# boromir674/relation-autoencoder

Measured on NVIDIA B200. Metric: AC-model train examples/sec, higher is better.
Workload: dtype f32

## Files before the change

### relation_autoencoder_b200/csrc/rae_decoder_tc.cu

```cuda
#include <cuda_fp16.h>
#include <stdlib.h>

#include <algorithm>
#include <vector>

#include "rae_common.cuh"
#include "rae_internal.h"

namespace rae {

namespace {

#ifdef RAE_TRACE
__device__ unsigned long long* g_tc_trace = nullptr;
__device__ int g_tc_knock = 0;
#define TC_KNOCK(bit) ((g_tc_knock & (bit)) != 0)
#define TC_TRACE_INIT() unsigned long long* const tc_trace_ptr_ = g_tc_trace
#define TC_TRACE_INIT_IF(cond) unsigned long long* const tc_trace_ptr_ = (cond) ? g_tc_trace : nullptr
#define TC_TRACE(slot)                                                                                         \
    do {                                                                                                       \
        if (tc_trace_ptr_ != nullptr && (slot) < 64) tc_trace_ptr_[(size_t)blockIdx.x * 64 + (slot)] = clock64(); \
    } while (0)
#define TC_TRACE_NS(slot)                                                                                      \
    do {                                                                                                       \
// ... 168 lines not shown
    asm volatile("tcgen05.st.sync.aligned.32x32b.x4.b32 [%0], {%1, %2, %3, %4};" ::"r"(taddr), "r"(v[0]), "r"(v[1]), "r"(v[2]), "r"(v[3])
                 : "memory");
}
__host__ __device__ __forceinline__ float pow2_scale(uint32_t amax_bits) {
    const int e = (int)((amax_bits >> 23) & 255u) - 127;
    if (((amax_bits >> 23) & 255u) == 0u) return 1.f;
    int se = 11 - e;
    se = se < -100 ? -100 : (se > 100 ? 100 : se);
    union { uint32_t u; float f; } cv;
    cv.u = (uint32_t)(se + 127) << 23;
    return cv.f;
}
constexpr float TC_QSCALE = 4096.f;
enum TcScal { TS_AMAX_C = 0, TS_AMAX_L = 1, TS_AMAX_R = 2, TS_AMAX_A = 3, TS_AMAX_CV = 4, TS_AMAX_Y2 = 5, TS_N = 8 };

__device__ __forceinline__ float ldg_stream(const float* p) {
    float v;
    asm volatile("ld.global.nc.f32 %0, [%1];" : "=f"(v) : "l"(p));
    return v;
}

__device__ __forceinline__ float ldg_ordered(const float* p) {
    float v;
    asm volatile("ld.global.f32 %0, [%1];" : "=f"(v) : "l"(p) : "memory");
    return v;
}

struct TcSeg { int tile, u0, u1, slot; };
struct TcSegIter {
    TcSched s; long long cur, end; int x;
    __device__ __forceinline__ TcSegIter(TcSched s_, int x_) : s(s_), cur(tcs_start(s_, x_)), end(tcs_start(s_, x_ + 1)), x(x_) {}
    __device__ __forceinline__ bool next(TcSeg& g) {
        if (cur >= end) return false;
        g.tile = (int)(cur / s.upt);
        g.u0 = (int)(cur - (long long)g.tile * s.upt);
        const long long len = min((long long)(s.upt - g.u0), end - cur);
        g.u1 = g.u0 + (int)len;
        g.slot = x - tcs_first(s, g.tile);
        cur += len;
        return true;
    }
};

__device__ __forceinline__ const float* cf_row(const float* C, const float* C1, const float* C2, int d, int K, int DP,
                                               int n_bil_rows, int n) {
    if (n < n_bil_rows) {
        const int i = n / DP, j = n - i * DP;
        return (i < d && j < d && C != nullptr) ? C + ((size_t)i * d + j) * K : nullptr;
    }
    const int m = n - n_bil_rows;
    const int which = m / DP, j = m - which * DP;
    if (j >= d || which > 1) return nullptr;
    const float* src = which == 0 ? C1 : C2;
    return src != nullptr ? src + (size_t)j * K : nullptr;
}

__global__ void __launch_bounds__(256) k_tc_absmax(const float* __restrict__ C, size_t nC, const float* __restrict__ C1, size_t n1,
                                                   const float* __restrict__ C2, size_t n2, uint32_t* __restrict__ out) {
    pdl_enter();
    __shared__ uint32_t red[8];
    uint32_t m = 0;
    const size_t stride = (size_t)gridDim.x * blockDim.x, t0 = (size_t)blockIdx.x * blockDim.x + threadIdx.x;
    auto scan = [&](const float* p, size_t n) {
        if (p == nullptr || n == 0) return;
        if ((n & 3) == 0 && (reinterpret_cast<uintptr_t>(p) & 15) == 0) {
            const float4* p4 = reinterpret_cast<const float4*>(p);
// ... 377 lines not shown
                        for (int x = 0; x < 32; ++x)
                            if (jb + x < p.d) o[(size_t)(jb + x) * p.B] = inv * t[x];
                    }
                }
                if (DP >= 64 && bil && ok && i0 < p.d) p.vT[((size_t)g * p.dp + i0) * p.B + b] = inv * vsum;
                if (etr) TC_TRACE(56);
            }
            if (ok) {
                float* wo = p.wT + ((size_t)sg.slot * 2 + g) * p.dp * p.B + b;
#pragma unroll
                for (int c = 0; c < RW; ++c) {
                    const int j = jbase + c;
                    if (j < p.dp) wo[(size_t)j * p.B] = inv * Wr[c];
                }
            }
            if (ew == 0 && lane == 0 && it <= (sg.u1 - sg.u0)) TC_TRACE(9);
        }
        if (ew == 0 && lane == 0) TC_TRACE(4);
    }
    tc_fence_before();
    __syncthreads();
    if (threadIdx.x == 0) { TC_TRACE(5); TC_TRACE_NS(15); }
    if (warp == TC_FWD_WORKERS + 2) {
        tc_fence_after();
        asm volatile("tcgen05.dealloc.cta_group::1.sync.aligned.b32 %0, %1;" ::"r"(tmem_base), "r"(512u) : "memory");
    }
}

constexpr uint32_t TC_BWD_ACOL = 128;
constexpr int TC_DQ_ASTAGES = 3;
constexpr int TC_DC_ASTAGES = 2;
constexpr uint32_t TC_BWD_ACC2 = 384;
constexpr int TC_DC_MAX_STAGES = 16;
constexpr int TC_DQ_MAX_STAGES = 64;

constexpr int TC_IMG_LD = 68;
struct TrJob { const float* src; size_t stride; int cols, cols_out; float* dst; uint32_t* amax; int img; };
struct TrJobs { TrJob j[4]; int B; };
__global__ void __launch_bounds__(256) k_tc_transpose(TrJobs jobs) {
    pdl_enter();
    __shared__ float tile[32][33];
    __shared__ uint32_t red[8];
    const TrJob jb = jobs.j[blockIdx.z];
    const int b0 = blockIdx.x * 32, c0 = blockIdx.y * 32;
    if (c0 >= jb.cols_out) return;
    const int tx = threadIdx.x & 31, ty = threadIdx.x >> 5;
    uint32_t m = 0;
    for (int r = ty; r < 32; r += 8) {
        const int b = b0 + r, c = c0 + tx;
        const float v = (b < jobs.B && c < jb.cols) ? jb.src[(size_t)b * jb.stride + c] : 0.f;
        tile[r][tx] = v;
        m = max(m, __float_as_uint(fabsf(v)));
    }
    if (jb.amax != nullptr) {
#pragma unroll
        for (int o = 16; o > 0; o >>= 1) m = max(m, __shfl_xor_sync(kFull, m, o));
        if (tx == 0) red[ty] = m;
    }
    __syncthreads();
    for (int r = ty; r < 32; r += 8) {
        const int c = c0 + r, b = b0 + tx;
        if (c < jb.cols_out && b < jobs.B) {
            if (jb.img) jb.dst[((size_t)(b >> 6) * jb.cols_out + c) * TC_IMG_LD + (b & 63)] = tile[tx][r];
            else jb.dst[(size_t)c * jobs.B + b] = tile[tx][r];
        }
    }
    if (jb.amax != nullptr && threadIdx.x == 0) {
// ... 127 lines not shown
            tc_commit(&br.b_empty[s]);
            if (lt == nst - 1) tc_commit(br.acc_full);
        }
        __syncwarp();
        if ((threadIdx.x & 31) == 0 && git == 8) TC_TRACE(trace_base + 7);
        if ((threadIdx.x & 31) == 0 && git == 24) TC_TRACE(trace_base + 12);
    }
}

__device__ __forceinline__ void bwd_store8(uint32_t lane_base, int as, int col8, const float (&g)[8]) {
    float hi[8], lo[8];
    split8(g, hi, lo);
    const uint32_t col = lane_base + TC_BWD_ACOL + 128u * as + (uint32_t)col8;
    tc_st8(col, hi);
    tc_st8(col + 64u, lo);
}
__device__ __forceinline__ void bwd_publish(const BwdBars& br, int as, int lane) {
    tc_wait_st();
    tc_fence_before();
    __syncwarp();
    if (lane == 0) mbar_arrive(&br.a_full[as]);
}

struct TcDqArgs {
    const uint4* bop2;
    const float* sc;
    const float* aT; const float* LT; const float* RT; const float* cT; const float* Y2T;
    float* dqT;
    const uint32_t* scal;
    float g_bound;
    int B, d, dp, K, NK;
    int n_bil_rows;
    TcSched sch;
};

__device__ __forceinline__ void dq_mma_segment(const BwdBars& br, uint8_t* smB, uint32_t ST_BYTES, int NK, uint32_t tmem_base, int nst,
                                               int it0) {
    TC_TRACE_INIT();
    constexpr int NAS = TC_DQ_ASTAGES;
    const uint32_t idesc = make_idesc_f16(TC_M, NK);
    bool ready = false;
    for (int lt = 0; lt < nst; ++lt) {
        const int git = it0 + lt, s = git % TC_BSTAGES, as = git % NAS;
        if (!ready) {
            mbar_wait(&br.a_full[as], (git / NAS) & 1);
            mbar_wait(&br.b_full[s], (git / TC_BSTAGES) & 1);
            tc_fence_after();
        }
        ready = false;
        if (git == 8) TC_TRACE(22);
        if (git == 24) TC_TRACE(27);
        const uint32_t a_hi = tmem_base + TC_BWD_ACOL + 128u * as, a_lo = a_hi + 64u;
        const uint32_t b_base = smem_u32(smB + (size_t)s * ST_BYTES);
        uint64_t dbh = make_desc(b_base, (uint32_t)NK * 16u, 128u);
        uint64_t dbl = make_desc(b_base + 16u * (uint32_t)NK * 16u, (uint32_t)NK * 16u, 128u);
#pragma unroll
        for (int ks = 0; ks < 8; ++ks) {
            if (TC_KNOCK(2)) continue;
            if (ks == 4 && lt + 1 < nst) {
                const int g1 = git + 1;
                mbar_wait(&br.a_full[g1 % NAS], (g1 / NAS) & 1);
                mbar_wait(&br.b_full[g1 % TC_BSTAGES], (g1 / TC_BSTAGES) & 1);
                tc_fence_after();
                ready = true;
            }
            tc_mma_f16_ts(tmem_base, a_hi + 8u * ks, dbh, idesc, (lt > 0 || ks > 0) ? 1u : 0u);
// ... 9 lines not shown
        if (git == 24) TC_TRACE(28);
    }
}

__device__ __forceinline__ void dq_store16(uint32_t lane_base, int as, int col8, const float (&g)[16]) {
    uint32_t hi[8], lo[8];
#pragma unroll
    for (int u = 0; u < 8; ++u) split_h2(g[2 * u], g[2 * u + 1], hi[u], lo[u]);
    const uint32_t col = lane_base + TC_BWD_ACOL + 128u * as + (uint32_t)col8;
    tc_st8u(col, hi);
    tc_st8u(col + 64u, lo);
}

template <int DP>
__global__ void __launch_bounds__(TC_BWD_THREADS, 1) k_tc_dq(TcDqArgs p) {
    pdl_enter();
    extern __shared__ __align__(128) uint8_t smem_raw[];
    const int warp = threadIdx.x >> 5, lane = threadIdx.x & 31;
    TC_TRACE_INIT();
    constexpr int NAS = TC_DQ_ASTAGES;
    constexpr int RPS = 128 / DP;
    const uint32_t ST_BYTES = 2u * 16u * (uint32_t)p.NK * 16u;
    uint8_t* smB = smem_raw;
    uint32_t tmem_base;
    if (threadIdx.x == 0) { TC_TRACE(16); TC_TRACE_NS(30); }
    const BwdBars br = bwd_setup(smem_raw, ST_BYTES, warp, tmem_base);
    if (threadIdx.x == 0) TC_TRACE(17);

    if (warp >= TC_BWD_WORKERS) {
        asm volatile("setmaxnreg.dec.sync.aligned.u32 32;" ::: "memory");
    }
    if (warp == TC_BWD_WORKERS + 1) {
        if (lane == 0) {
            TcSegIter si(p.sch, blockIdx.x);
            TcSeg sg;
            int it = 0;
            while (si.next(sg)) {
                bwd_produce(br, smB, reinterpret_cast<const uint8_t*>(p.bop2), ST_BYTES, sg.u0, sg.u1 - sg.u0, it);
                it += sg.u1 - sg.u0;
            }
        }
    } else if (warp == TC_BWD_WORKERS) {
        if (elect_one()) {
            TcSegIter si(p.sch, blockIdx.x);
            TcSeg sg;
            int it = 0, seg = 0;
            while (si.next(sg)) {
                if (seg > 0) {
                    mbar_wait(br.acc_empty, (seg - 1) & 1);
                    tc_fence_after();
                }
                dq_mma_segment(br, smB, ST_BYTES, p.NK, tmem_base, sg.u1 - sg.u0, it);
                it += sg.u1 - sg.u0;
                ++seg;
            }
            TC_TRACE(19);
        }
        __syncwarp();
    } else if (warp < TC_BWD_WORKERS) {
        asm volatile("setmaxnreg.inc.sync.aligned.u32 112;" ::: "memory");
        const int gw = warp, q4 = gw & 3, cg = gw >> 2;
        const int row = q4 * 32 + lane;
        const uint32_t lane_base = tmem_base + ((uint32_t)(q4 * 32) << 16);
        const int rsel = (32 * cg) / DP, j0 = (32 * cg) % DP;
        const int n_bil_st = p.n_bil_rows / TC_M;
        float sG, inv;
        {
            const float aL = __uint_as_float(p.scal[TS_AMAX_L]), aR = __uint_as_float(p.scal[TS_AMAX_R]);
            const float aA = __uint_as_float(p.scal[TS_AMAX_A]), aC = __uint_as_float(p.scal[TS_AMAX_CV]);
            const float aY = __uint_as_float(p.scal[TS_AMAX_Y2]);
            const float bound = fmaxf(fmaf(aA, aR, aL * aY), fmaxf(fmaf(p.g_bound, aL, aA), fmaf(p.g_bound, aR, aC)));
            sG = pow2_scale(__float_as_uint(bound));
            inv = 1.f / (sG * pow2_scale(p.scal[TS_AMAX_C]));
        }
        TcSegIter si(p.sch, blockIdx.x);
        TcSeg sg;
        int it = 0, seg = 0;
        while (si.next(sg)) {
            const int b = sg.tile * TC_M + row;
            const bool ok = b < p.B;
            const float* scb = p.sc + (size_t)(ok ? b : 0) * SC_N;
            float X[32], Y[32];
            {
                const float* rp = p.RT + (ok ? b : 0);
                const float* yp = p.Y2T + (ok ? b : 0);
                const int jlast = p.dp - 1;
#pragma unroll
                for (int u = 0; u < 32; ++u) {
                    X[u] = ldg_stream(rp + (size_t)min(j0 + u, jlast) * p.B);
                    Y[u] = ldg_stream(yp + (size_t)min(j0 + u, jlast) * p.B);
                }
#pragma unroll
                for (int u = 0; u < 32; ++u)
                    if (!(ok && j0 + u < p.dp)) { X[u] = 0.f; Y[u] = 0.f; }
            }
            if (gw == 0 && lane == 0 && it == 0 && X[0] != -1.f) TC_TRACE(29);
            const int st0 = sg.u0, st1 = sg.u1, nst = st1 - st0;
            const int nbil = max(0, min(st1, n_bil_st) - st0);
            float ai_n = 0.f, li_n = 0.f;
            {
                const int i = RPS * st0 + rsel;
                if (nbil > 0 && ok && i < p.dp) {
                    ai_n = p.aT[(size_t)i * p.B + b];
                    li_n = p.LT[(size_t)i * p.B + b];
                }
            }
            int lt = 0;
            for (; lt < nbil; ++lt) {
// ... 686 lines not shown
    for (int j = lane; j < d; j += 32) {
        o[E_L * dp + j] = ld_nc(A + (size_t)r1 * d + j);
        o[E_R * dp + j] = ld_nc(A + (size_t)r2 * d + j);
    }
}
}

int tc_supported(const rae_engine* h) {
    if (!h->hasM) return 0;
    if (h->d <= 16 || h->d > 128) return 0;
    if (h->K > 104) return 0;
    return 1;
}

int tc_init(rae_engine* h) {
    const int DP = tc_dp(h->d);
    TcState& t = h->tc;
    t.DP = DP;
    t.KH = (h->K + 15) & ~15;
    const int rps = 128 / DP;
    const int di = (h->d + rps - 1) / rps * rps;
    t.n_bil_rows = di * DP;
    t.n_bil_half = t.n_bil_rows / TC_H;
    t.n_sp_half = h->hasSP ? (2 * DP) / TC_H : 0;
    t.n_rows_total = (t.n_bil_rows + (h->hasSP ? 2 * DP : 0) + TC_M - 1) / TC_M * TC_M;
    t.n_chunks_fwd = (t.n_bil_half + t.n_sp_half + 1) / 2;
    t.n_chunks_rec = t.n_bil_half / 2;
    t.ntile = (h->B + TC_M - 1) / TC_M;
    const size_t b_bytes = (size_t)2 * (t.KH / 8) * TC_N * 16;
    t.fwd_stages = (int)std::min<size_t>(4, ((size_t)h->max_smem_optin - 256) / b_bytes);
    if (t.fwd_stages < 2) return fail(h, RAE_EINVAL, "tensor path: K=%d needs %zu bytes per operand stage, two do not fit", h->K, b_bytes);
    t.smem = (size_t)t.fwd_stages * b_bytes + 256;
    t.sch_fwd = make_sched(t.ntile, t.n_chunks_fwd, h->num_sms, 0);
    t.sch_rec = make_sched(t.ntile, t.n_chunks_rec, h->num_sms, 0);
    t.slots_vw = std::max(sched_max_slots(t.sch_fwd), sched_max_slots(t.sch_rec));
    t.NK = (h->K + 15) & ~15;
    const int n_st = t.n_rows_total / TC_M;
    t.sch_dq = make_sched(t.ntile, n_st, h->num_sms, TC_DQ_MAX_STAGES);
    t.slots_dq = sched_max_slots(t.sch_dq);
    const size_t st_bytes = (size_t)2 * 2 * 8 * t.NK * 16;
    t.smem_dq = (size_t)TC_BSTAGES * st_bytes + 256;
    if (t.smem_dq > (size_t)h->max_smem_optin) return fail(h, RAE_EINVAL, "tensor path: backward operand stages do not fit in shared memory");
    t.n_ntiles = t.n_rows_total / TC_M;
    t.n_bst = (h->B + TC_SR - 1) / TC_SR;
    t.dc_nacc = 2;
    const size_t per_stage = (size_t)(TC_M / DP) * 2 * TC_SR * sizeof(float);
    const int cap = (int)(((size_t)h->max_smem_optin - t.smem_dq) / per_stage);
    if (cap < 1) return fail(h, RAE_EINVAL, "tensor path: no shared memory left for the dC staging area");
    const int n_bil_tiles = t.n_bil_rows / TC_M;
    t.dc2 = (h->B % 4 == 0) && n_bil_tiles > 0;
    t.smem_dc2 = (size_t)TC_DC2_BSTAGES * (2 * 8 * t.NK * 16) + (size_t)TC_DC2_XSTAGES * (2 * (size_t)DP * TC_IMG_LD * 4 + 2 * (TC_M / DP) * 2 * 256) + 256;
    if (t.smem_dc2 > (size_t)h->max_smem_optin) t.dc2 = false;
    t.dc_tile0 = t.dc2 ? n_bil_tiles : 0;
    t.slots_dc = 1;
    if (t.dc2) {
        t.sch_dc2 = make_sched((n_bil_tiles + 1) / 2, t.n_bst, h->num_sms, TC_DC2_MAX_STAGES);
        t.slots_dc = sched_max_slots(t.sch_dc2);
    }
    t.dc_tiles = t.n_ntiles - t.dc_tile0;
    if (t.dc_tiles > 0) {
        t.sch_dc = make_sched(t.dc_tiles, t.n_bst, h->num_sms, std::min(t.dc_nacc * TC_DC_MAX_STAGES, cap));
        t.dc_share = sched_max_share(t.sch_dc);
        t.slots_dc = std::max(t.slots_dc, sched_max_slots(t.sch_dc));
    }
    t.smem_dc = t.smem_dq + (size_t)t.dc_share * per_stage;
    cudaError_t e;
    const size_t vec = (size_t)h->dp * h->B * sizeof(float);
    if ((e = cudaMalloc((void**)&t.bop, (size_t)t.n_chunks_fwd * b_bytes)) != cudaSuccess ||
        (e = cudaMalloc((void**)&t.vT, 2 * vec)) != cudaSuccess ||
        (e = cudaMalloc((void**)&t.wT, 2 * t.slots_vw * vec)) != cudaSuccess ||
        (e = cudaMalloc((void**)&t.spT, 2 * vec)) != cudaSuccess ||
// ... 90 lines not shown
                                                              h->quirk ? 1 : 0, h->ev, t.scal, reinterpret_cast<uint4*>(t.pop4));
    h->launches++;
    RAE_CUDA(h, cudaGetLastError());
    const int slots[2] = {E_L, E_R};
    float* const dst[2] = {t.LT, t.RT};
    const int words[2] = {TS_AMAX_L, TS_AMAX_R};
    return tc_transpose_slots(h, 2, slots, dst, words, true, E_R, t.Rimg, st);
}

int tc_prepare_qt(rae_engine* h, cudaStream_t st) {
    TcState& t = h->tc;
    const int nbc = 2 * t.n_bst;
    const size_t total3 = (size_t)nbc * 8 * t.NK;
    const int blocks3 = (int)std::min<size_t>((total3 + 255) / 256, (size_t)h->num_sms * 8);
    launch_pdl(k_tc_prep_qt, dim3(blocks3, 1), dim3(256), 0, st, h->q, h->B, h->K, t.NK, nbc, t.pop3, h->P[RAE_P_A], nullptr, nullptr, h->d, h->dp,
                                                   h->quirk ? 1 : 0, h->ev, t.scal, nullptr);
    h->launches++;
    RAE_CUDA(h, cudaGetLastError());
    return RAE_OK;
}

int tc_contract(rae_engine* h, const float* LT_in, const float* RT_in, int slotV, int slotW, bool with_sp, cudaStream_t st) {
    TcState& t = h->tc;
    TcArgs p{};
    p.qT = t.qT; p.bop = t.bop; p.LT = LT_in; p.RT = RT_in; p.spT = t.spT; p.vT = t.vT; p.wT = t.wT; p.scal = t.scal;
    p.B = h->B; p.K = h->K; p.d = h->d; p.dp = h->dp; p.KH = t.KH;
    p.n_bil_half = t.n_bil_half; p.n_sp_half = with_sp ? t.n_sp_half : 0;
    p.nbs = t.fwd_stages;
    p.sch = with_sp ? t.sch_fwd : t.sch_rec;
    if (t.DP == 32) launch_pdl(k_tc_bilinear<32>, dim3(p.sch.G), dim3(TC_FWD_THREADS), t.smem, st, p);
    else if (t.DP == 64) launch_pdl(k_tc_bilinear<64>, dim3(p.sch.G), dim3(TC_FWD_THREADS), t.smem, st, p);
    else launch_pdl(k_tc_bilinear<128>, dim3(p.sch.G), dim3(TC_FWD_THREADS), t.smem, st, p);
    RAE_CUDA(h, cudaGetLastError());
    launch_pdl(k_tc_combine, dim3((h->B + 31) / 32, (h->d + 31) / 32), dim3(256), 0, st, t.vT, t.wT, (with_sp && h->hasSP) ? t.spT : nullptr, h->ev, h->B, h->d,
                                                                          h->dp, t.DP, p.sch, slotV, slotW, with_sp ? t.scal : nullptr);
    h->launches += 2;
    RAE_CUDA(h, cudaGetLastError());
    return RAE_OK;
}

int tc_forward(rae_engine* h, cudaStream_t st) { return tc_contract(h, h->tc.LT, h->tc.RT, E_V1, E_V2, true, st); }

int tc_backward_recompute(rae_engine* h, cudaStream_t st) {
    TcState& t = h->tc;
    const int slots[3] = {E_A, E_CV, E_Y2};
    float* const dst[3] = {t.aT, t.cT, t.Y2T};
    const int words[3] = {TS_AMAX_A, TS_AMAX_CV, TS_AMAX_Y2};
    int rc = tc_transpose_slots(h, 3, slots, dst, words, false, E_Y2, t.Yimg, st);
    if (rc) return rc;
    return tc_contract(h, t.aT, t.cT, E_GA1, E_GA2, false, st);
}

int tc_backward_dq(rae_engine* h, cudaStream_t st) {
    TcState& t = h->tc;
    TcDqArgs p{};
    p.bop2 = reinterpret_cast<const uint4*>(t.bop2); p.sc = h->sc; p.aT = t.aT; p.LT = t.LT; p.RT = t.RT; p.cT = t.cT; p.Y2T = t.Y2T;
    p.dqT = t.dqT; p.scal = t.scal; p.g_bound = (float)((double)h->S / h->Z);
    p.B = h->B; p.d = h->d; p.dp = h->dp; p.K = h->K; p.NK = t.NK;
    p.n_bil_rows = t.n_bil_rows;
    p.sch = t.sch_dq;
    if (t.DP == 32) launch_pdl(k_tc_dq<32>, dim3(p.sch.G), dim3(TC_BWD_THREADS), t.smem_dq, st, p);
    else if (t.DP == 64) launch_pdl(k_tc_dq<64>, dim3(p.sch.G), dim3(TC_BWD_THREADS), t.smem_dq, st, p);
    else launch_pdl(k_tc_dq<128>, dim3(p.sch.G), dim3(TC_BWD_THREADS), t.smem_dq, st, p);
    h->launches += 1;
    RAE_CUDA(h, cudaGetLastError());
    return RAE_OK;
}

int tc_backward_finish(rae_engine* h, cudaStream_t st) {
    TcState& t = h->tc;
    const int blocks = (h->B + 31) / 32;
    if (blocks > h->n_dz_part) return fail(h, RAE_EINVAL, "internal: dzsum_part too small");
    h->dz_part_used = blocks;
    const size_t smem = sizeof(float) * 32 * ((size_t)(h->K | 1) + h->K);
    launch_pdl(k_tc_bwd_finish, dim3(blocks), dim3(1024), smem, st, h->ev, h->sc, h->q, h->logq, t.dqT, h->dz, h->dzsum_part, h->B, h->K, t.NK, t.sch_dq,
                                               h->d, h->dp, h->hasSP ? 1 : 0, (float)(2.0 * h->cfg.alpha / h->Z));
    h->launches += 1;
    RAE_CUDA(h, cudaGetLastError());
    return RAE_OK;
}

int tc_grad_dense(rae_engine* h, cudaStream_t st) {
    TcState& t = h->tc;
    if (t.dc2) {
        TcDc2Args p{};
        p.pop4 = reinterpret_cast<const uint4*>(t.pop4); p.Rimg = t.Rimg; p.Yimg = t.Yimg; p.aT = t.aT; p.LT = t.LT; p.out = h->gC_part;
        p.scal = t.scal; p.g_bound = (float)((double)h->S / h->Z);
        p.B = h->B; p.d = h->d; p.dp = h->dp; p.K = h->K; p.NK = t.NK; p.DP = t.DP;
        p.n_bil_tiles = t.n_bil_rows / TC_M;
        p.split_stride = (size_t)h->off_gWb;
        p.sch = t.sch_dc2;
        launch_pdl(k_tc_dc2, dim3(p.sch.G), dim3(TC_BWD_THREADS), t.smem_dc2, st, p);
        h->launches++;
        RAE_CUDA(h, cudaGetLastError());
    }
    if (t.dc_tiles > 0) {
// ... 391 lines not shown
```

### relation_autoencoder_b200/csrc/rae_engine.cu

```cuda
#include <stdarg.h>
#include <stdlib.h>
#include <string.h>

#include <new>
#include <vector>

#include "rae_internal.h"

namespace rae {

bool g_pdl_enabled = true;

static char g_create_err[512] = "";

int fail(rae_engine* h, int code, const char* fmt, ...) {
    va_list ap;
    va_start(ap, fmt);
    char* dst = h ? h->err : g_create_err;
    vsnprintf(dst, 512, fmt, ap);
    va_end(ap);
    return code;
}

template <typename T>
// ... 430 lines not shown
        const int max_by_batch = (h->B + 63) / 64;
        if (ns > max_by_batch) ns = max_by_batch;
        if (ns < 1) ns = 1;
        if (h->use_tc) ns = h->tc.slots_dc;
        h->gC_nsplit = ns;
        RAE_CREATE_RC(dev_alloc(h, &h->gC_part, (size_t)ns * (size_t)(dd + 2 * dk)));
    }
    if (h->dense_w || h->debug_dense || h->emit_only) RAE_CREATE_RC(dev_alloc(h, &h->gW_dense, (size_t)cfg->F * h->K));
    if (h->debug_dense || h->emit_only) {
        RAE_CREATE_RC(dev_alloc(h, &h->gA_dense, (size_t)cfg->N * h->d));
        RAE_CREATE_RC(dev_alloc(h, &h->gAb_dense, (size_t)cfg->N));
    }
    h->own_gW = h->gW_dense; h->own_gA = h->gA_dense; h->own_gAb = h->gAb_dense; h->own_dense = h->dense_grad;
    const int64_t n_occ = (int64_t)(2 + 2 * h->S) * h->B;
    RAE_CREATE_RC(alloc_segwork(h, h->ent, n_occ, bits_for(cfg->N)));
    RAE_CREATE_RC(ensure_cub(h, n_occ));
    h->ent_cub_bytes = segwork_temp_bytes(n_occ);
    RAE_CREATE_CUDA(cudaMalloc(&h->ent_cub_tmp, h->ent_cub_bytes));
    RAE_CREATE_CUDA(cudaStreamCreateWithFlags(&h->s1, cudaStreamNonBlocking));
    RAE_CREATE_CUDA(cudaStreamCreateWithFlags(&h->s2, cudaStreamNonBlocking));
    RAE_CREATE_CUDA(cudaEventCreateWithFlags(&h->ev_fork0, cudaEventDisableTiming));
    RAE_CREATE_CUDA(cudaEventCreateWithFlags(&h->ev_fork1, cudaEventDisableTiming));
    RAE_CREATE_CUDA(cudaEventCreateWithFlags(&h->ev_join1, cudaEventDisableTiming));
    RAE_CREATE_CUDA(cudaEventCreateWithFlags(&h->ev_join2, cudaEventDisableTiming));
    RAE_CREATE_CUDA(cudaEventCreateWithFlags(&h->ev_prepc, cudaEventDisableTiming));
    RAE_CREATE_CUDA(cudaEventCreateWithFlags(&h->ev_q, cudaEventDisableTiming));
    RAE_CREATE_CUDA(cudaEventCreateWithFlags(&h->ev_qt, cudaEventDisableTiming));
    RAE_CREATE_CUDA(cudaEventCreateWithFlags(&h->ev_dfork, cudaEventDisableTiming));
    RAE_CREATE_CUDA(cudaEventCreateWithFlags(&h->ev_dfetch, cudaEventDisableTiming));
    RAE_CREATE_CUDA(cudaEventCreateWithFlags(&h->ev_score, cudaEventDisableTiming));
    RAE_CREATE_CUDA(cudaEventCreateWithFlags(&h->ev_cost, cudaEventDisableTiming));
    RAE_CREATE_CUDA(cudaEventCreateWithFlags(&h->ev_neg, cudaEventDisableTiming));
    RAE_CREATE_CUDA(cudaEventCreateWithFlags(&h->ev_gcost, cudaEventDisableTiming));
    RAE_CREATE_RC(dev_alloc(h, &h->stage_neg, 4 * (size_t)(h->S > 0 ? h->S : 1) * h->B));
    RAE_CREATE_CUDA(cudaMallocHost((void**)&h->pinned_neg, sizeof(int32_t) * 2 * (size_t)(h->S > 0 ? h->S : 1) * h->B));
    RAE_CREATE_RC(dev_alloc(h, &h->peer_err_dev, 1));
    RAE_CREATE_CUDA(cudaMemset(h->peer_err_dev, 0, sizeof(int32_t)));
    RAE_CREATE_RC(dev_alloc(h, &h->stat_dev, 2));
    RAE_CREATE_CUDA(cudaMemset(h->stat_dev, 0, 2 * sizeof(int32_t)));
    RAE_CREATE_RC(dev_alloc(h, &h->label_dev, (size_t)h->B));
    RAE_CREATE_RC(dev_alloc(h, &h->prob_dev, BK));
#undef RAE_CREATE_CUDA
#undef RAE_CREATE_RC
    *out = h;
    return RAE_OK;
}

void rae_destroy(rae_engine* h) {
    if (!h) return;
    cudaFree(h->q); cudaFree(h->logq); cudaFree(h->dz); cudaFree(h->ev); cudaFree(h->sc); cudaFree(h->gn1); cudaFree(h->gn2);
    cudaFree(h->loss_part); cudaFree(h->reg_part); cudaFree(h->cost_dev); cudaFree(h->dzsum_part); cudaFree(h->own_dense);
    cudaFree(h->gC_part); cudaFree(h->own_gW); cudaFree(h->own_gA); cudaFree(h->own_gAb); cudaFree(h->cub_tmp);
    cudaFree(h->ent_part); cudaFree(h->feat_part); cudaFree(h->stat_dev); cudaFree(h->peer_err_dev);
    cudaFree(h->stage_neg); cudaFree(h->label_dev); cudaFree(h->prob_dev);
    if (h->ev_created) {
        for (int i = 0; i <= RAE_NUM_PHASES; ++i) cudaEventDestroy(h->ev_phase[i]);
        for (int i = 0; i < 3; ++i) cudaEventDestroy(h->ev_upd[i]);
    }
    cudaFree(h->push.w_dev);
    if (h->tl_created) {
        for (int i = 0; i < RAE_TL_MAX; ++i) cudaEventDestroy(h->tl_ev[i]);
    }
    if (h->s1) cudaStreamDestroy(h->s1);
    if (h->s2) cudaStreamDestroy(h->s2);
    if (h->ev_fork0) cudaEventDestroy(h->ev_fork0);
    if (h->ev_fork1) cudaEventDestroy(h->ev_fork1);
    if (h->ev_join1) cudaEventDestroy(h->ev_join1);
    if (h->ev_join2) cudaEventDestroy(h->ev_join2);
    if (h->ev_score) cudaEventDestroy(h->ev_score);
    if (h->ev_cost) cudaEventDestroy(h->ev_cost);
    if (h->ev_neg) cudaEventDestroy(h->ev_neg);
    if (h->ev_gcost) cudaEventDestroy(h->ev_gcost);
    if (h->ev_prepc) cudaEventDestroy(h->ev_prepc);
    if (h->ev_q) cudaEventDestroy(h->ev_q);
    if (h->ev_qt) cudaEventDestroy(h->ev_qt);
    if (h->ev_dfork) cudaEventDestroy(h->ev_dfork);
    if (h->ev_dfetch) cudaEventDestroy(h->ev_dfetch);
    cudaFree(h->ent_cub_tmp);
    if (h->cost_pinned) cudaFreeHost(h->cost_pinned);
    if (h->pinned_neg) cudaFreeHost(h->pinned_neg);
    free_segwork(h->ent);
    free_segwork(h->feat);
    free_feature_cache(h->fcache);
    tc_free(h);
    cudaGetLastError();
    delete h;
}

int rae_bind_params(rae_engine* h, float* W, float* Wb, float* A, float* Ab, float* C, float* C1, float* C2) {
    if (!h) return RAE_EINVAL;
    if (!W || !Wb || !A || !Ab) return fail(h, RAE_EINVAL, "rae_bind_params: W, Wb, A, Ab must be non-null");
    if (h->hasM && !C) return fail(h, RAE_EINVAL, "rae_bind_params: this model needs C (R) [d,d,K]");
    if (h->hasSP && (!C1 || !C2)) return fail(h, RAE_EINVAL, "rae_bind_params: this model needs C1 and C2 [d,K]");
    float* v[RAE_NUM_PARAMS] = {W, Wb, A, Ab, C, C1, C2};
    for (int i = 0; i < RAE_NUM_PARAMS; ++i) h->P[i] = v[i];
    h->params_bound = true;
    return RAE_OK;
}

int rae_bind_accumulators(rae_engine* h, float* W, float* Wb, float* A, float* Ab, float* C, float* C1, float* C2) {
    if (!h) return RAE_EINVAL;
    if (!Wb || (!h->emit_only && (!W || !A || !Ab)))
        return fail(h, RAE_EINVAL, "rae_bind_accumulators: W, Wb, A, Ab must be non-null (W, A, Ab may be NULL with RAE_FLAG_EMIT_ONLY)");
    if (h->hasM && !C) return fail(h, RAE_EINVAL, "rae_bind_accumulators: this model needs C (R) [d,d,K]");
    if (h->hasSP && (!C1 || !C2)) return fail(h, RAE_EINVAL, "rae_bind_accumulators: this model needs C1 and C2 [d,K]");
// ... 327 lines not shown
```

### relation_autoencoder_b200/csrc/rae_internal.h

```cpp
#pragma once
#include <cuda_runtime.h>
#include <stdint.h>
#include <stdio.h>

#include "../../include/rae.h"

namespace rae {

enum EvSlot {
    E_L = 0,
    E_R = 1,
    E_V1 = 2,
    E_V2 = 3,
    E_C1 = 4,
    E_C2 = 5,
    E_A = 6,
    E_CV = 7,
    E_Y2 = 8,
    E_GA1 = 9,
    E_GA2 = 10,
    E_NV = 11
};
enum ScSlot { SC_GU1 = 0, SC_GU2 = 1, SC_GP = 2, SC_G1 = 3, SC_G2 = 4, SC_ENT = 5, SC_N = 8 };

// ... 30 lines not shown
};

struct TcSched { int G, upt, ntile; };
__host__ __device__ __forceinline__ long long tcs_start(TcSched s, int x) { return (long long)x * s.upt * s.ntile / s.G; }
__host__ __device__ __forceinline__ int tcs_cta_of(TcSched s, long long u) {
    const long long T = (long long)s.upt * s.ntile;
    return (int)(((u + 1) * s.G + T - 1) / T) - 1;
}
__host__ __device__ __forceinline__ int tcs_first(TcSched s, int tile) { return tcs_cta_of(s, (long long)tile * s.upt); }
__host__ __device__ __forceinline__ int tcs_nslots(TcSched s, int tile) {
    if (s.G == 0) return s.upt;
    return tcs_cta_of(s, (long long)(tile + 1) * s.upt - 1) - tcs_first(s, tile) + 1;
}

struct TcState {
    bool ready = false;
    int DP = 0;
    int KH = 0;
    int n_bil_rows = 0, n_bil_half = 0, n_sp_half = 0;
    int n_rows_total = 0;
    int n_chunks_fwd = 0;
    int n_chunks_rec = 0;
    int ntile = 0;
    int fwd_stages = 2;
    size_t smem = 0;
    TcSched sch_fwd{}, sch_rec{}, sch_dq{}, sch_dc{}, sch_dc2{};
    int slots_vw = 0, slots_dq = 0, slots_dc = 0;
    float4* bop = nullptr;
    float* vT = nullptr;
    float* wT = nullptr;
    float* spT = nullptr;
    uint32_t* scal = nullptr;
    int NK = 0; size_t smem_dq = 0, smem_dc = 0;
    float4* bop2 = nullptr;
    float* dqT = nullptr;
    int n_ntiles = 0, n_bst = 0, dc_nacc = 2, dc_share = 0;
    bool dc2 = false; int dc_tile0 = 0, dc_tiles = 0; size_t smem_dc2 = 0;
    float4* pop4 = nullptr; float* Rimg = nullptr; float* Yimg = nullptr;
    int32_t* tile_slots = nullptr;
    float4* pop3 = nullptr;
    float* qT = nullptr;
    float* aT = nullptr; float* LT = nullptr; float* RT = nullptr; float* cT = nullptr; float* Y2T = nullptr;
};

}

constexpr int RAE_TL_MAX = 48;
struct rae_engine {
    rae_config cfg;
    int K, d, S, B;
    int dp;
    bool hasM, hasSP, quirk, adagrad, debug_dense, emit_only;
    bool reg;
    bool dense_w;
    double Z;
    float* P[RAE_NUM_PARAMS];
    float* ACC[RAE_NUM_PARAMS];
    bool params_bound, acc_bound;
    rae::SplitBinding split[RAE_NUM_SPLITS];
    const int32_t* neg1;
    const int32_t* neg2;
    int64_t neg_cols;

    float* q;
    float* logq;
    float* dz;
    float* ev;
    float* sc;
    float* gn1;
    float* gn2;
    double* loss_part; int n_loss_part;
    double* reg_part;  int n_reg_part;
    double* cost_dev;
    double* cost_pinned;
    float* dzsum_part; int n_dz_part; int dz_part_used;
    float* dense_grad;
    int64_t off_gC, off_gC1, off_gC2, off_gWb, n_dense;
    bool dense_fused;
    float* gC_part; int gC_nsplit;
    float* gW_dense; float* gA_dense; float* gAb_dense;
    float* own_gW; float* own_gA; float* own_gAb; float* own_dense;
    rae::SegWork ent, feat;
    float* ent_part; size_t ent_part_cap;
    float* feat_part; size_t feat_part_cap;
    rae::FeatureCache fcache;
    rae::TcState tc; bool use_tc;
    void* cub_tmp; size_t cub_bytes;
    void* ent_cub_tmp; size_t ent_cub_bytes;
    cudaStream_t s1, s2;
    cudaEvent_t ev_fork0, ev_fork1, ev_join1, ev_join2, ev_prepc, ev_dfork, ev_dfetch, ev_q, ev_qt;
    cudaEvent_t ev_score, ev_cost, ev_neg, ev_gcost;
    double* gcost_pinned;
    int32_t* neg_err_pinned;
    bool gcost_pending;
    cudaEvent_t neg_wait;
    bool cost_on_event;
    bool neg_staged;
    bool neg_direct;
    int stage_flip;
    int barrier_epoch, barrier_epoch1; int32_t* peer_err_dev;
    int32_t* peer_err_pinned;
    cudaEvent_t pending_wait;
    int32_t* stage_neg;
    int32_t* pinned_neg;
    int64_t* label_dev; float* prob_dev;
    rae_step_stats stats;
    bool profiling; cudaEvent_t ev_phase[RAE_NUM_PHASES + 1]; cudaEvent_t ev_upd[3]; bool ev_created;
    struct { float** w_dev; float** a_dev; float** ab_dev; int world, rank; int64_t f_cap, n_cap; bool on;
             const int32_t* f_ids; const int32_t* e_ids; } push;
    void* dense_wait;
    bool tl_keep;
    bool timeline; int tl_n; cudaEvent_t tl_ev[RAE_TL_MAX]; const char* tl_name[RAE_TL_MAX]; int tl_stream[RAE_TL_MAX]; bool tl_created;
    const uint32_t* last_f_keys_s; int64_t last_f_n;
    int32_t* stat_dev;
    int launches;
    int num_sms;
    bool coop_launch;
    int max_smem_optin;
    char err[512];
};

namespace rae {

int fail(rae_engine* h, int code, const char* fmt, ...);
#define RAE_CUDA(h, expr)                                                                          \
    do {                                                                                           \
        cudaError_t _e = (expr);                                                                   \
        if (_e != cudaSuccess)                                                                     \
            return rae::fail((h), RAE_ECUDA, "%s failed at %s:%d: %s", #expr, __FILE__, __LINE__, \
                             cudaGetErrorString(_e));                                              \
    } while (0)

int launch_encoder_forward(rae_engine* h, const int32_t* indptr, const int32_t* indices, int B, float* q, float* logq,
                           float* sc_ent , int64_t* labels, cudaStream_t st);
int launch_label_shards(rae_engine* h, const void* const* w_shards, int world, const int32_t* indptr, const int32_t* indices,
                        int64_t n_rows, int64_t* labels, float* probs, cudaStream_t st);
int launch_label_topk(rae_engine* h, const void* const* w_shards, int world, const int32_t* indptr, const int32_t* indices,
                      int64_t n_rows, int k, int32_t* ids, float* probs, cudaStream_t st);

int simt_supported(const rae_engine* h, char* why, size_t n);
int launch_bilinear_forward_simt(rae_engine* h, const int32_t* a1, const int32_t* a2, cudaStream_t st);
int launch_score(rae_engine* h, const int32_t* a1, const int32_t* a2, const int32_t* neg1, const int32_t* neg2,
                 int64_t neg_ld, cudaStream_t st);
int launch_bilinear_backward_simt(rae_engine* h, cudaStream_t st);
int launch_grad_dense_simt(rae_engine* h, cudaStream_t st);

int tc_supported(const rae_engine* h);
int tc_init(rae_engine* h);
void tc_free(rae_engine* h);
int tc_prepare_c(rae_engine* h, cudaStream_t st);
int tc_prepare_p(rae_engine* h, const int32_t* a1, const int32_t* a2, cudaStream_t st);
int tc_prepare_qt(rae_engine* h, cudaStream_t st);
int tc_gather_lr(rae_engine* h, const int32_t* a1, const int32_t* a2, cudaStream_t st);
int tc_forward(rae_engine* h, cudaStream_t st);
int tc_backward_recompute(rae_engine* h, cudaStream_t st);
int tc_backward_dq(rae_engine* h, cudaStream_t st);
int tc_backward_finish(rae_engine* h, cudaStream_t st);
int tc_grad_dense(rae_engine* h, cudaStream_t st);
int launch_rank_arguments(rae_engine* h, const int32_t* indptr, const int32_t* indices, const int32_t* a1, const int32_t* a2,
                          int64_t n_rows, int32_t* rank1, int32_t* rank2, cudaStream_t st);

size_t segwork_temp_bytes(int64_t n);
constexpr int64_t RAE_OWN_SORT_MAX = 1 << 20;
size_t radix_sort_temp_bytes(int64_t n, int num_sms);
int radix_sort_pairs(rae_engine* h, const uint32_t* keys, const uint32_t* vals, uint32_t* keys_s, uint32_t* vals_s, int64_t n,
                     int key_bits, cudaStream_t st, void* tmp, size_t tmp_bytes);
int radix_sort_entities(rae_engine* h, const int32_t* a1, const int32_t* a2, const int32_t* neg1, const int32_t* neg2,
                        int64_t neg_ld, uint32_t* keys_s, uint32_t* vals_s, int key_bits, cudaStream_t st, void* tmp,
                        size_t tmp_bytes);
int sort_entities(rae_engine* h, const int32_t* a1, const int32_t* a2, const int32_t* neg1, const int32_t* neg2, int64_t neg_ld,
                  cudaStream_t st);
int build_entity_keys(rae_engine* h, const int32_t* a1, const int32_t* a2, const int32_t* neg1, const int32_t* neg2,
                      int64_t neg_ld, cudaStream_t st);
int build_feature_keys(rae_engine* h, const int32_t* indptr, const int32_t* indices, cudaStream_t st);
int sort_pairs(rae_engine* h, SegWork& w, int64_t n, cudaStream_t st, void* tmp, size_t tmp_bytes);
int segment_heads(rae_engine* h, const uint32_t* keys_s, int64_t n, SegWork& w, cudaStream_t st);
int count_unique(rae_engine* h, const uint32_t* keys_s, int64_t n, int32_t* out_dev, cudaStream_t st);
int build_feature_cache(rae_engine* h, cudaStream_t st);
int launch_entity_update(rae_engine* h, const uint32_t* keys_s, const uint32_t* vals_s, int64_t n_occ, bool emit_dense,
                         bool apply, cudaStream_t st);
int launch_w_update(rae_engine* h, const uint32_t* keys_s, const uint32_t* vals_s, int64_t nnz, bool emit_dense,
                    bool apply, cudaStream_t st);
int launch_fetch_rows(rae_engine* h, const void* const* tables, int world, int64_t width, const int32_t* ids, int64_t n,
                      float* out, cudaStream_t st);
int launch_pull_apply(rae_engine* h, float* table, float* acc, int64_t width, const int32_t* rows_local, const int32_t* ent_off,
                      const int32_t* ent_src, const int32_t* ent_slot, int64_t n_rows, const void* const* grads, int world,
                      cudaStream_t st);
int launch_shard_apply(rae_engine* h, float* table, float* acc, int64_t width, const int32_t* rows_local, const int32_t* ent_off,
                       const int32_t* ent_src, const int32_t* ent_slot, int64_t n_rows, const void* const* grads, int world,
// ... 12 lines not shown
```

Before: 8.899 million.

## Run backward dQ kernel concurrently with recompute contraction on split SMs

```diff
diff --git a/relation_autoencoder_b200/csrc/rae_decoder_tc.cu b/relation_autoencoder_b200/csrc/rae_decoder_tc.cu
--- a/relation_autoencoder_b200/csrc/rae_decoder_tc.cu
+++ b/relation_autoencoder_b200/csrc/rae_decoder_tc.cu
@@ -224,6 +224,26 @@
     __device__ __forceinline__ TcSegIter(TcSched s_, int x_) : s(s_), cur(tcs_start(s_, x_)), end(tcs_start(s_, x_ + 1)), x(x_) {}
     __device__ __forceinline__ bool next(TcSeg& g) {
         if (cur >= end) return false;
+        g.tile = (int)(cur / s.upt);
+        g.u0 = (int)(cur - (long long)g.tile * s.upt);
+        const long long len = min((long long)(s.upt - g.u0), end - cur);
+        g.u1 = g.u0 + (int)len;
+        g.slot = x - tcs_first(s, g.tile);
+        cur += len;
+        return true;
+    }
+};
+
+struct TcSegRange {
+    TcSched s; long long cur, end; int x, x1;
+    __device__ __forceinline__ TcSegRange(TcSched s_, int x0, int x1_)
+        : s(s_), cur(tcs_start(s_, x0)), end(x0 < min(x1_, s_.G) ? tcs_start(s_, x0 + 1) : tcs_start(s_, x0)), x(x0), x1(min(x1_, s_.G)) {}
+    __device__ __forceinline__ bool next(TcSeg& g) {
+        while (cur >= end) {
+            if (x + 1 >= x1) return false;
+            ++x;
+            end = tcs_start(s, x + 1);
+        }
         g.tile = (int)(cur / s.upt);
         g.u0 = (int)(cur - (long long)g.tile * s.upt);
         const long long len = min((long long)(s.upt - g.u0), end - cur);
@@ -667,7 +687,7 @@
 constexpr int TC_DC_ASTAGES = 2;
 constexpr uint32_t TC_BWD_ACC2 = 384;
 constexpr int TC_DC_MAX_STAGES = 16;
-constexpr int TC_DQ_MAX_STAGES = 64;
+constexpr int TC_DQ_MAX_STAGES = 28;
 
 constexpr int TC_IMG_LD = 68;
 struct TrJob { const float* src; size_t stride; int cols, cols_out; float* dst; uint32_t* amax; int img; };
@@ -861,6 +881,7 @@
     int B, d, dp, K, NK;
     int n_bil_rows;
     TcSched sch;
+    int vpc;
 };
 
 __device__ __forceinline__ void dq_mma_segment(const BwdBars& br, uint8_t* smB, uint32_t ST_BYTES, int NK, uint32_t tmem_base, int nst,
@@ -936,7 +957,7 @@
     }
     if (warp == TC_BWD_WORKERS + 1) {
         if (lane == 0) {
-            TcSegIter si(p.sch, blockIdx.x);
+            TcSegRange si(p.sch, (int)blockIdx.x * p.vpc, ((int)blockIdx.x + 1) * p.vpc);
             TcSeg sg;
             int it = 0;
             while (si.next(sg)) {
@@ -946,7 +967,7 @@
         }
     } else if (warp == TC_BWD_WORKERS) {
         if (elect_one()) {
-            TcSegIter si(p.sch, blockIdx.x);
+            TcSegRange si(p.sch, (int)blockIdx.x * p.vpc, ((int)blockIdx.x + 1) * p.vpc);
             TcSeg sg;
             int it = 0, seg = 0;
             while (si.next(sg)) {
@@ -977,7 +998,7 @@
             sG = pow2_scale(__float_as_uint(bound));
             inv = 1.f / (sG * pow2_scale(p.scal[TS_AMAX_C]));
         }
-        TcSegIter si(p.sch, blockIdx.x);
+        TcSegRange si(p.sch, (int)blockIdx.x * p.vpc, ((int)blockIdx.x + 1) * p.vpc);
         TcSeg sg;
         int it = 0, seg = 0;
         while (si.next(sg)) {
@@ -1730,11 +1751,16 @@
     if (t.fwd_stages < 2) return fail(h, RAE_EINVAL, "tensor path: K=%d needs %zu bytes per operand stage, two do not fit", h->K, b_bytes);
     t.smem = (size_t)t.fwd_stages * b_bytes + 256;
     t.sch_fwd = make_sched(t.ntile, t.n_chunks_fwd, h->num_sms, 0);
-    t.sch_rec = make_sched(t.ntile, t.n_chunks_rec, h->num_sms, 0);
-    t.slots_vw = std::max(sched_max_slots(t.sch_fwd), sched_max_slots(t.sch_rec));
     t.NK = (h->K + 15) & ~15;
     const int n_st = t.n_rows_total / TC_M;
-    t.sch_dq = make_sched(t.ntile, n_st, h->num_sms, TC_DQ_MAX_STAGES);
+    const long long u_rec = (long long)t.ntile * t.n_chunks_rec, u_dq = (long long)t.ntile * n_st;
+    int sms_rec = (int)((h->num_sms * u_rec + (u_rec + u_dq) / 2) / (u_rec + u_dq));
+    sms_rec = std::max(1, std::min(sms_rec, h->num_sms - 1));
+    t.sch_rec = make_sched(t.ntile, t.n_chunks_rec, sms_rec, 0);
+    t.slots_vw = std::max(sched_max_slots(t.sch_fwd), sched_max_slots(t.sch_rec));
+    const int sms_dq = std::max(1, h->num_sms - sms_rec);
+    t.sch_dq = make_sched(t.ntile, n_st, sms_dq, TC_DQ_MAX_STAGES);
+    t.dq_vpc = (t.sch_dq.G + sms_dq - 1) / sms_dq;
     t.slots_dq = sched_max_slots(t.sch_dq);
     const size_t st_bytes = (size_t)2 * 2 * 8 * t.NK * 16;
     t.smem_dq = (size_t)TC_BSTAGES * st_bytes + 256;
@@ -1891,8 +1917,14 @@
     else if (t.DP == 64) launch_pdl(k_tc_bilinear<64>, dim3(p.sch.G), dim3(TC_FWD_THREADS), t.smem, st, p);
     else launch_pdl(k_tc_bilinear<128>, dim3(p.sch.G), dim3(TC_FWD_THREADS), t.smem, st, p);
     RAE_CUDA(h, cudaGetLastError());
-    launch_pdl(k_tc_combine, dim3((h->B + 31) / 32, (h->d + 31) / 32), dim3(256), 0, st, t.vT, t.wT, (with_sp && h->hasSP) ? t.spT : nullptr, h->ev, h->B, h->d,
-                                                                          h->dp, t.DP, p.sch, slotV, slotW, with_sp ? t.scal : nullptr);
+    const dim3 cgrid((h->B + 31) / 32, (h->d + 31) / 32);
+    const float* spT = (with_sp && h->hasSP) ? t.spT : nullptr;
+    uint32_t* zero_amax = with_sp ? t.scal : nullptr;
+    if (with_sp) {
+        launch_pdl(k_tc_combine, cgrid, dim3(256), 0, st, t.vT, t.wT, spT, h->ev, h->B, h->d, h->dp, t.DP, p.sch, slotV, slotW, zero_amax);
+    } else {
+        k_tc_combine<<<cgrid, 256, 0, st>>>(t.vT, t.wT, spT, h->ev, h->B, h->d, h->dp, t.DP, p.sch, slotV, slotW, zero_amax);
+    }
     h->launches += 2;
     RAE_CUDA(h, cudaGetLastError());
     return RAE_OK;
@@ -1907,10 +1939,19 @@
     const int words[3] = {TS_AMAX_A, TS_AMAX_CV, TS_AMAX_Y2};
     int rc = tc_transpose_slots(h, 3, slots, dst, words, false, E_Y2, t.Yimg, st);
     if (rc) return rc;
+    RAE_CUDA(h, cudaEventRecord(h->ev_bwd_fork, st));
+    RAE_CUDA(h, cudaStreamWaitEvent(h->s2, h->ev_bwd_fork, 0));
+    if ((rc = tc_backward_dq_launch(h, h->s2))) return rc;
+    RAE_CUDA(h, cudaEventRecord(h->ev_bwd_join, h->s2));
     return tc_contract(h, t.aT, t.cT, E_GA1, E_GA2, false, st);
 }
 
 int tc_backward_dq(rae_engine* h, cudaStream_t st) {
+    RAE_CUDA(h, cudaStreamWaitEvent(st, h->ev_bwd_join, 0));
+    return RAE_OK;
+}
+
+int tc_backward_dq_launch(rae_engine* h, cudaStream_t st) {
     TcState& t = h->tc;
     TcDqArgs p{};
     p.bop2 = reinterpret_cast<const uint4*>(t.bop2); p.sc = h->sc; p.aT = t.aT; p.LT = t.LT; p.RT = t.RT; p.cT = t.cT; p.Y2T = t.Y2T;
@@ -1918,9 +1959,11 @@
     p.B = h->B; p.d = h->d; p.dp = h->dp; p.K = h->K; p.NK = t.NK;
     p.n_bil_rows = t.n_bil_rows;
     p.sch = t.sch_dq;
-    if (t.DP == 32) launch_pdl(k_tc_dq<32>, dim3(p.sch.G), dim3(TC_BWD_THREADS), t.smem_dq, st, p);
-    else if (t.DP == 64) launch_pdl(k_tc_dq<64>, dim3(p.sch.G), dim3(TC_BWD_THREADS), t.smem_dq, st, p);
-    else launch_pdl(k_tc_dq<128>, dim3(p.sch.G), dim3(TC_BWD_THREADS), t.smem_dq, st, p);
+    p.vpc = t.dq_vpc;
+    const dim3 grid((p.sch.G + p.vpc - 1) / p.vpc);
+    if (t.DP == 32) launch_pdl(k_tc_dq<32>, grid, dim3(TC_BWD_THREADS), t.smem_dq, st, p);
+    else if (t.DP == 64) launch_pdl(k_tc_dq<64>, grid, dim3(TC_BWD_THREADS), t.smem_dq, st, p);
+    else launch_pdl(k_tc_dq<128>, grid, dim3(TC_BWD_THREADS), t.smem_dq, st, p);
     h->launches += 1;
     RAE_CUDA(h, cudaGetLastError());
     return RAE_OK;
diff --git a/relation_autoencoder_b200/csrc/rae_engine.cu b/relation_autoencoder_b200/csrc/rae_engine.cu
--- a/relation_autoencoder_b200/csrc/rae_engine.cu
+++ b/relation_autoencoder_b200/csrc/rae_engine.cu
@@ -486,6 +486,8 @@
     RAE_CREATE_CUDA(cudaEventCreateWithFlags(&h->ev_cost, cudaEventDisableTiming));
     RAE_CREATE_CUDA(cudaEventCreateWithFlags(&h->ev_neg, cudaEventDisableTiming));
     RAE_CREATE_CUDA(cudaEventCreateWithFlags(&h->ev_gcost, cudaEventDisableTiming));
+    RAE_CREATE_CUDA(cudaEventCreateWithFlags(&h->ev_bwd_fork, cudaEventDisableTiming));
+    RAE_CREATE_CUDA(cudaEventCreateWithFlags(&h->ev_bwd_join, cudaEventDisableTiming));
     RAE_CREATE_RC(dev_alloc(h, &h->stage_neg, 4 * (size_t)(h->S > 0 ? h->S : 1) * h->B));
     RAE_CREATE_CUDA(cudaMallocHost((void**)&h->pinned_neg, sizeof(int32_t) * 2 * (size_t)(h->S > 0 ? h->S : 1) * h->B));
     RAE_CREATE_RC(dev_alloc(h, &h->peer_err_dev, 1));
@@ -525,6 +527,8 @@
     if (h->ev_cost) cudaEventDestroy(h->ev_cost);
     if (h->ev_neg) cudaEventDestroy(h->ev_neg);
     if (h->ev_gcost) cudaEventDestroy(h->ev_gcost);
+    if (h->ev_bwd_fork) cudaEventDestroy(h->ev_bwd_fork);
+    if (h->ev_bwd_join) cudaEventDestroy(h->ev_bwd_join);
     if (h->ev_prepc) cudaEventDestroy(h->ev_prepc);
     if (h->ev_q) cudaEventDestroy(h->ev_q);
     if (h->ev_qt) cudaEventDestroy(h->ev_qt);
diff --git a/relation_autoencoder_b200/csrc/rae_internal.h b/relation_autoencoder_b200/csrc/rae_internal.h
--- a/relation_autoencoder_b200/csrc/rae_internal.h
+++ b/relation_autoencoder_b200/csrc/rae_internal.h
@@ -86,6 +86,7 @@
     float* spT = nullptr;
     uint32_t* scal = nullptr;
     int NK = 0; size_t smem_dq = 0, smem_dc = 0;
+    int dq_vpc = 1;
     float4* bop2 = nullptr;
     float* dqT = nullptr;
     int n_ntiles = 0, n_bst = 0, dc_nacc = 2, dc_share = 0;
@@ -144,6 +145,7 @@
     cudaStream_t s1, s2;
     cudaEvent_t ev_fork0, ev_fork1, ev_join1, ev_join2, ev_prepc, ev_dfork, ev_dfetch, ev_q, ev_qt;
     cudaEvent_t ev_score, ev_cost, ev_neg, ev_gcost;
+    cudaEvent_t ev_bwd_fork, ev_bwd_join;
     double* gcost_pinned;
     int32_t* neg_err_pinned;
     bool gcost_pending;
@@ -209,6 +211,7 @@
 int tc_forward(rae_engine* h, cudaStream_t st);
 int tc_backward_recompute(rae_engine* h, cudaStream_t st);
 int tc_backward_dq(rae_engine* h, cudaStream_t st);
+int tc_backward_dq_launch(rae_engine* h, cudaStream_t st);
 int tc_backward_finish(rae_engine* h, cudaStream_t st);
 int tc_grad_dense(rae_engine* h, cudaStream_t st);
 int launch_rank_arguments(rae_engine* h, const int32_t* indptr, const int32_t* indices, const int32_t* a1, const int32_t* a2,
```

New measurement: 9.301 million (median of 6 runs). 4.5% higher.
